# NILOIDE/A.I.gar

Measured on NVIDIA B200. Metric: env_steps_per_sec, higher is better.
Workload: dtype f64

## Files before the change

a.i.gar_b200/csrc/agar_b200.cu:

```cuda
#include <cuda_runtime.h>
#include <math.h>
#include <stdio.h>
#include <stdlib.h>
#include <string.h>

#include "../../include/agar_b200.h"
#include "../../include/agar_layout.h"
#include "agar_bots.cuh"
#include "agar_dev.cuh"
#include "agar_simple.cuh"

extern __shared__ __align__(16) uint8_t g_smem[];

__device__ __forceinline__ void stage_in(const DevParams& P, const uint8_t* state, int env0, int n_here, bool zero) {
    const int chunks = (int)(P.L.record_bytes / 8);
    const int total = n_here * chunks;
    const uint2* src = (const uint2*)(state + (size_t)env0 * P.L.record_bytes);
    for (int i = threadIdx.x; i < total; i += blockDim.x) {
        int e = i / chunks, w = i - e * chunks;
        uint2 v = zero ? make_uint2(0u, 0u) : src[i];
        ((uint2*)(g_smem + (size_t)e * P.rec_stride))[w] = v;
    }
    __syncthreads();
}
// ... 139 lines not shown
            CLK_MARK(1);
            c.fov_done = false, c.n_live = -1;
            for (int ph = 0; ph < AGAR_FIELD_PHASES; ++ph) {
                if (ph == 0 ? psync : psync_field) __syncthreads();
                if (ph == 0) CLK_MARK(2);
                if (active) field_update_phase<W, FULL>(c, P, ph);
                CLK_MARK(3 + ph);
            }
            if (active) {
                if (c.lane == 0) c.h->frame += 1;
                c.t.sync();
            }
            CLK_MARK(12);
        }
        if (active && c.lane == 0 && (P.turn_reward || P.turn_done))
            for (int a = 0; a < A; ++a) {
                if (P.turn_reward) P.turn_reward[(size_t)env * A + a] = (float)c.pl[a].bot.last_reward;
                if (P.turn_done) P.turn_done[(size_t)env * A + a] = (uint8_t)c.pl[a].bot.exp_done;
            }
    }
    if (P.stage == 1) stage_out(P, state, env0, n_here);
    if (P.stage >= 2) {
        __syncthreads();
        pel_cache_copy(P, state, env0, n_here, tiles, false);
    }
    export_tail(P, obs, env0, n_here);
}


struct SimplePlan {
    int frame_sync;
    int strideB;
    int grid_off;
};
template <int W>
__global__ void __launch_bounds__(256, W == 1 ? 2 : 1)
k_simple(const __grid_constant__ DevParams P, const SimplePlan SP, uint8_t* __restrict__ state, const float* __restrict__ actions,
         float* __restrict__ obs, int n_frames, int n_dec, int flags, uint32_t dec_base) {
    const int per = blockDim.x / W;
    const int env0 = blockIdx.x * per;
    const int n_here = min(per, P.n_envs - env0);
    const int rec_words = (int)(P.L.record_bytes / 4), pel_word = (int)(P.L.off_pellets / 4);
    const int tail_words = rec_words - pel_word;
    {
        for (int i = threadIdx.x; i < per * tail_words; i += blockDim.x) {
            int e = i / tail_words, w = i - e * tail_words;
            int es = e < n_here ? e : n_here - 1;
            const uint32_t* src = (const uint32_t*)(state + (size_t)(env0 + es) * P.L.record_bytes) + pel_word;
            *(uint32_t*)(g_smem + (size_t)e * SP.strideB + w * 4) = src[w];
        }
    }
    __syncthreads();
    const int slot = threadIdx.x / W, sub = threadIdx.x % W;
    const bool valid = slot < n_here;
    const int env = env0 + (valid ? slot : n_here - 1);
    const uint32_t env_id = (uint32_t)(P.first_env + (uint64_t)env);
    uint8_t* rec = state + (size_t)env * P.L.record_bytes;
    uint8_t* b = g_smem + (size_t)slot * SP.strideB;
    SPtr q;
    q.h = (AgarEnvHeader*)(rec + P.L.off_header);
    q.p = (AgarPlayer*)(rec + P.L.off_players);
    q.c = (AgarCell*)(rec + P.L.off_cells);
    q.pel = (uint32_t*)b;
    q.ev = (AgarEvent*)(b + (P.L.off_events - P.L.off_pellets));
    q.grid = SP.grid_off ? (uint32_t*)(b + SP.grid_off) : nullptr;
    SReg r;
    s_load(r, q);
    float* row = (obs != nullptr && valid) ? obs + (size_t)env * P.L.state_len : nullptr;
    for (int d = 0; d < n_dec; ++d) {
        if (flags & KF_OBS_BEFORE) {
            int d_o = s_turn_begin(r, P);
            s_observe<W>(r, q, P, d_o != 0, row, sub);
        }
        for (int f = 0; f < n_frames; ++f) {
            if (SP.frame_sync == 1 || SP.frame_sync == 4) __syncthreads();
            if (SP.frame_sync == 2) __syncwarp();
            r.n_events = 0;
            int d_o = s_turn_begin(r, P);
            s_observe<W>(r, q, P, d_o != 0, nullptr, sub);
            float act[4] = {0.f, 0.f, 0.f, 0.f};
            if (r.need_action) {
                if (flags & KF_RANDOM_ACTIONS) {
                    uint32_t w[4];
                    philox(dec_base + (uint32_t)d, 7u, env_id, 0u, (uint32_t)P.seed, (uint32_t)(P.seed >> 32), w);
                    for (int i = 0; i < 4; ++i) act[i] = (float)(w[i] >> 8) * (1.0f / 16777216.0f);
                } else {
                    const float* ap = actions + (size_t)env * 4;
                    for (int i = 0; i < 4; ++i) act[i] = ap[i];
                }
            }
            double speed_pow;
            s_turn_end<W>(r, P, act, sub, speed_pow);
            if (SP.frame_sync == 4) __syncthreads();
            s_field_update<W>(r, q, P, env_id, sub, speed_pow);
        }
    }
    if (flags & KF_OBS_AFTER) {
        int d_o = s_turn_begin(r, P);
        s_observe<W>(r, q, P, d_o != 0, row, sub);
    }
    if (valid && sub == 0) {
        s_store(r, q);
        if (P.turn_reward) P.turn_reward[env] = (float)r.last_reward;
        if (P.turn_done) P.turn_done[env] = (uint8_t)r.exp_done;
    }
    __syncthreads();
    for (int i = threadIdx.x; i < n_here * tail_words; i += blockDim.x) {
        int e = i / tail_words, w = i - e * tail_words;
        uint32_t* dst = (uint32_t*)(state + (size_t)(env0 + e) * P.L.record_bytes) + pel_word;
        dst[w] = *(const uint32_t*)(g_smem + (size_t)e * SP.strideB + w * 4);
    }
    export_tail(P, obs, env0, n_here);
}

template <int W, bool FULL>
__global__ void __launch_bounds__(1024)
k_init(const __grid_constant__ DevParams P, uint8_t* __restrict__ state, const uint8_t* __restrict__ mask, int mode) {
    const int tiles = blockDim.x / W;
    const int env0 = blockIdx.x * tiles;
    const int n_here = min(tiles, P.n_envs - env0);
    if (P.stage == 1)
        stage_in(P, state, env0, n_here, mode == 0);
    else if (mode == 0) {
        const int chunks = (int)(P.L.record_bytes / 8);
        uint2* dst = (uint2*)(state + (size_t)env0 * P.L.record_bytes);
        for (int i = threadIdx.x; i < n_here * chunks; i += blockDim.x) dst[i] = make_uint2(0u, 0u);
        __syncthreads();
    }
    if (P.stage >= 2) pel_cache_copy(P, state, env0, n_here, tiles, true);
    const int tile_id = threadIdx.x / W;
    if (tile_id < n_here && (mask == nullptr || mode == 0 || mask[env0 + tile_id])) {
        Ctx<W> c(cg::tiled_partition<W>(cg::this_thread_block()));
        bind_ctx(c, P, tile_id, tiles, env0 + tile_id, state);
        const int K = P.L.n_players;
        if (mode == 0 || mode == 1) {
            if (mode == 1) {
                for (int i = c.lane; i < P.L.pellet_cap; i += W) c.pel[i] = 0;
// ... 64 lines not shown
    case AGAR_GET_VALID: ((uint8_t*)out)[i] = (uint8_t)p->bot.exp_valid; break;
    case AGAR_GET_NEED_ACTION: ((uint8_t*)out)[i] = (uint8_t)p->bot.need_action; break;
    case AGAR_GET_MASS: {
        int nc = p->n_cells;
        ((float*)out)[i] = nc ? (float)np_sum([&](int j) { return cells[j].mass; }, nc) : 0.f;
        break;
    }
    case AGAR_GET_FOV: ((float*)out)[i] = (float)p->fov_size; break;
    case AGAR_GET_NCELLS: ((int32_t*)out)[i] = p->n_cells; break;
    case AGAR_GET_ALIVE: ((uint8_t*)out)[i] = (uint8_t)p->alive; break;
    case AGAR_GET_STATS: {
        double* o = (double*)out + (size_t)i * 4;
        o[0] = p->bot.stat_mass_sum, o[1] = p->bot.stat_mass_max, o[2] = p->bot.stat_frames, o[3] = p->bot.stat_deaths;
        break;
    }
    case AGAR_GET_OVERFLOW: ((uint32_t*)out)[i] = h->overflow; break;
    case AGAR_GET_EVENT_HASH: ((uint64_t*)out)[i] = h->event_hash; break;
    }
}

struct AgarEnv {
    AgarConfig cfg;
    AgarLayout L;
    DevParams P;
    uint8_t* state;
    double* deg_tab;
    int n_envs, device, W, full, threads, tiles;
    size_t smem_bytes;
    int init_W, init_threads, init_tiles;
    size_t init_smem;
    SimplePlan sp;
    int simple_W, simple_threads;
    size_t simple_smem;
    int64_t launches;
    char err[256];
    float *d_actions, *d_obs, *d_reward;
    uint8_t* d_done;
    void* h_turn;
    volatile uint32_t* h_flag;
    unsigned int* d_export_count;
    uint32_t flag_seq;
    int host_polling;
    int host_pending;
    int host_zerocopy;
};
static char g_create_err[256] = "";

static int fail(AgarEnv* e, int code, const char* fmt, const char* detail) {
    char* dst = e ? e->err : g_create_err;
    snprintf(dst, 256, fmt, detail);
    return code;
}
#define CU(call)                                                                 \
    do {                                                                         \
        cudaError_t _e = (call);                                                 \
        if (_e != cudaSuccess) return fail(env, AGAR_E_CUDA, "CUDA error: %s", cudaGetErrorString(_e)); \
    } while (0)

extern "C" int agar_layout_for_config(const AgarConfig* cfg, AgarLayout* out) {
    if (!cfg || !out) return AGAR_E_INVALID;
    return agar_layout_compute(cfg, out);
}

static bool config_is_simple(const AgarConfig& c, const AgarLayout& L) {
    return c.n_players == 1 && c.bot_type[0] == AGAR_BOT_NN && !c.virus_enabled && !c.enable_split && !c.enable_eject &&
           L.cell_cap == 1 && !c.self_grid && !c.wall_grid && !c.enemy_grid && !c.virus_grid && !c.self_grid_lf &&
           !c.self_grid_slf && !c.enemy_grid_lf && !c.enemy_grid_slf && !c.use_last_action && !c.use_second_last_action &&
// ... 52 lines not shown
    k_main<W, FULL, MAXT><<<blocks, e->threads, e->smem_bytes, s>>>(e->P, e->state, actions, obs, n_frames, n_dec, flags, dec_base);
    return cudaGetLastError();
}
template <int W, bool FULL>
static cudaError_t launch_main_t(AgarEnv* e, const float* actions, float* obs, int n_frames, int n_dec, int flags,
                                 uint32_t dec_base, cudaStream_t s) {
    if (W == 32 && FULL && e->threads > 768) return launch_main_k<32, true, 1024>(e, actions, obs, n_frames, n_dec, flags, dec_base, s);
    if (W == 32 && FULL && e->threads > 512) return launch_main_k<32, true, 768>(e, actions, obs, n_frames, n_dec, flags, dec_base, s);
    return launch_main_k<W, FULL, 512>(e, actions, obs, n_frames, n_dec, flags, dec_base, s);
}
template <int W, bool FULL>
static cudaError_t launch_init_t(AgarEnv* e, const uint8_t* mask, int mode, cudaStream_t s) {
    static unsigned char done[64];
    cudaError_t err = ensure_max_smem(k_init<W, FULL>, e->device, done);
    if (err != cudaSuccess) return err;
    int blocks = (e->n_envs + e->init_tiles - 1) / e->init_tiles;
    k_init<W, FULL><<<blocks, e->init_threads, e->init_smem, s>>>(e->P, e->state, mask, mode);
    return cudaGetLastError();
}
#define DISPATCH(fn, ...)                                                 \
    (e->full ? (e->W == 32  ? fn<32, true>(__VA_ARGS__)                   \
                : e->W == 16 ? fn<16, true>(__VA_ARGS__)                  \
                : e->W == 8  ? fn<8, true>(__VA_ARGS__)                   \
                             : fn<4, true>(__VA_ARGS__))                  \
             : (e->W == 32  ? fn<32, false>(__VA_ARGS__)                  \
                             : fn<32, false>(__VA_ARGS__)))

static int launch_main(AgarEnv* e, const float* actions, float* obs, int n_frames, int n_dec, int flags, uint32_t dec_base,
                       void* stream) {
    AgarEnv* env = e;
    CU(cudaSetDevice(e->device));
    cudaError_t err;
    if (e->simple_W) {
        int blocks = (e->n_envs * e->simple_W + e->simple_threads - 1) / e->simple_threads;
#define LAUNCH_SIMPLE(WW)                                                                                                     \
    do {                                                                                                                      \
        static unsigned char done_##WW[64];                                                                                   \
        err = ensure_max_smem(k_simple<WW>, e->device, done_##WW);                                                            \
        if (err == cudaSuccess) {                                                                                             \
            k_simple<WW><<<blocks, e->simple_threads, e->simple_smem, (cudaStream_t)stream>>>(e->P, e->sp, e->state, actions, obs, \
                                                                                              n_frames, n_dec, flags, dec_base);  \
            err = cudaGetLastError();                                                                                         \
        }                                                                                                                     \
    } while (0)
        if (e->simple_W == 1) LAUNCH_SIMPLE(1);
        else if (e->simple_W == 2) LAUNCH_SIMPLE(2);
        else if (e->simple_W == 4) LAUNCH_SIMPLE(4);
        else if (e->simple_W == 8) LAUNCH_SIMPLE(8);
        else if (e->simple_W == 16) LAUNCH_SIMPLE(16);
        else LAUNCH_SIMPLE(32);
#undef LAUNCH_SIMPLE
    } else
        err = DISPATCH(launch_main_t, e, actions, obs, n_frames, n_dec, flags, dec_base, (cudaStream_t)stream);
    if (err != cudaSuccess) return fail(e, AGAR_E_CUDA, "kernel launch failed: %s", cudaGetErrorString(err));
    e->launches += 1;
    return AGAR_OK;
}
static int launch_init(AgarEnv* e, const uint8_t* mask, int mode, void* stream) {
    AgarEnv* env = e;
    CU(cudaSetDevice(e->device));
    cudaError_t err = e->full ? (e->init_W == 32 ? launch_init_t<32, true>(e, mask, mode, (cudaStream_t)stream)
                                                  : launch_init_t<8, true>(e, mask, mode, (cudaStream_t)stream))
                              : launch_init_t<32, false>(e, mask, mode, (cudaStream_t)stream);
    if (err != cudaSuccess) return fail(e, AGAR_E_CUDA, "kernel launch failed: %s", cudaGetErrorString(err));
    e->launches += 1;
    return AGAR_OK;
}

extern "C" int agar_set_tile_width(AgarEnv* e, int W) {
    if (!e) return AGAR_E_INVALID;
    if (!e->full && e->L.grid_squares <= 16 && (W == 1 || W == 2 || W == 4 || W == 8 || W == 16 || W == 32) &&
        !getenv("AGAR_GENERAL_KERNEL")) {
        int tail_words = (int)((e->L.record_bytes - e->L.off_pellets) / 4);
        e->sp.strideB = (tail_words | 1) * 4;
        e->sp.grid_off = 0;
        const char* genv = getenv("AGAR_SIMPLE_OBS_SMEM");
        if (genv ? atoi(genv) != 0 : W >= 2) {
            const int gg = e->L.grid_squares * e->L.grid_squares;
            e->sp.grid_off = tail_words * 4;
            e->sp.strideB = ((tail_words + gg) | 1) * 4;
        }
        if (e->L.pellet_cap > (W >= 4 ? 64 : 128) * W)
            return fail(e, AGAR_E_UNSUPPORTED, "pellet pool too large for this tile width%s", "");
        int threads = 128;
        const char* tenv = getenv("AGAR_SIMPLE_THREADS");
        if (tenv && atoi(tenv) >= 32) threads = atoi(tenv) / 32 * 32;
        if (threads > 256) threads = 256;
        e->sp.frame_sync = getenv("AGAR_SIMPLE_SYNC") ? atoi(getenv("AGAR_SIMPLE_SYNC")) : 1;
        size_t per_env = (size_t)e->sp.strideB;
        while (threads > 32 && per_env * (threads / W) > 200 * 1024) threads -= 32;
        if (per_env * (threads / W) > 200 * 1024)
            return fail(e, AGAR_E_NOMEM, "pellet pool + event ring of %s do not fit in shared memory at this tile width", "the envs of one CTA");
        e->simple_W = W;
        e->simple_threads = threads;
        e->simple_smem = per_env * (threads / W);
        e->W = W;
        return AGAR_OK;
    }
    bool ok = W == 32 || (e->full && (W == 4 || W == 8 || W == 16));
    if (!ok) return fail(e, AGAR_E_INVALID, "unsupported tile width%s", "");
    if (!plan_launch(e, W)) return fail(e, AGAR_E_NOMEM, "env record does not fit in shared memory%s", "");
    e->simple_W = 0;
    return AGAR_OK;
}
extern "C" int agar_get_tile_width(const AgarEnv* e) { return e ? e->W : 0; }

extern "C" int agar_create(const AgarConfig* cfg, int n_envs, int device, uint64_t seed, uint64_t first_env_id, void* stream,
                           AgarEnv** out) {
    AgarEnv* env = nullptr;
    if (!cfg || !out || n_envs < 1) return fail(nullptr, AGAR_E_INVALID, "bad arguments to agar_create%s", "");
    AgarLayout L;
    int rc = agar_layout_compute(cfg, &L);
    if (rc != AGAR_OK) return fail(nullptr, rc, "config rejected by agar_layout_compute%s", "");
    int ndev = 0;
    if (cudaGetDeviceCount(&ndev) != cudaSuccess || device < 0 || device >= ndev)
        return fail(nullptr, AGAR_E_CUDA, "no such CUDA device%s", "");
    CU(cudaSetDevice(device));
    AgarEnv* e = (AgarEnv*)calloc(1, sizeof(AgarEnv));
    env = e;
    e->cfg = *cfg;
    e->L = L;
    e->n_envs = n_envs;
    e->device = device;
    e->full = config_is_simple(*cfg, L) ? 0 : 1;
    DevParams& P = e->P;
    memset(&P, 0, sizeof P);
    P.cfg = *cfg;
    P.L = L;
    P.S = L.field_size;
// ... 62 lines not shown
        cudaFree(e->state), cudaFree(e->deg_tab), free(e);
        return AGAR_E_NOMEM;
    }
    rc = launch_init(e, nullptr, 0, stream);
    if (rc != AGAR_OK) {
        snprintf(g_create_err, sizeof g_create_err, "%s", e->err);
        cudaFree(e->state), cudaFree(e->deg_tab), free(e);
        return rc;
    }
    *out = e;
    return AGAR_OK;
}
extern "C" int agar_destroy(AgarEnv* e) {
    if (!e) return AGAR_E_INVALID;
    cudaSetDevice(e->device);
    cudaFree(e->state);
    cudaFree(e->deg_tab);
    if (e->d_actions) cudaFree(e->d_actions);
    if (e->d_obs) cudaFree(e->d_obs);
    if (e->d_reward) cudaFree(e->d_reward);
    if (e->h_turn) cudaFreeHost(e->h_turn);
    if (e->d_export_count) cudaFree(e->d_export_count);
    free(e);
    return AGAR_OK;
}
extern "C" const char* agar_last_error(const AgarEnv* e) { return e ? e->err : g_create_err; }
extern "C" int agar_get_layout(const AgarEnv* e, AgarLayout* out) {
    if (!e || !out) return AGAR_E_INVALID;
    *out = e->L;
    return AGAR_OK;
}
extern "C" int agar_num_envs(const AgarEnv* e) { return e ? e->n_envs : AGAR_E_INVALID; }
extern "C" int64_t agar_launch_count(const AgarEnv* e) { return e ? e->launches : 0; }
extern "C" void* agar_state_ptr(const AgarEnv* e) { return e ? e->state : nullptr; }

extern "C" int agar_reset(AgarEnv* e, const uint8_t* env_mask_dev, void* stream) {
    if (!e) return AGAR_E_INVALID;
    return launch_init(e, env_mask_dev, 1, stream);
}
extern "C" int agar_reset_bots(AgarEnv* e, const uint8_t* env_mask_dev, void* stream) {
    if (!e) return AGAR_E_INVALID;
    return launch_init(e, env_mask_dev, 2, stream);
}
extern "C" int agar_observe(AgarEnv* e, float* obs_dev, void* stream) {
    if (!e) return AGAR_E_INVALID;
    return launch_main(e, nullptr, obs_dev, 0, 0, KF_OBS_AFTER, 0, stream);
}
extern "C" int agar_step(AgarEnv* e, const float* actions_dev, int n_frames, void* stream) {
    if (!e || n_frames < 0) return AGAR_E_INVALID;
    if (!actions_dev && e->L.n_agents > 0) return fail(e, AGAR_E_INVALID, "actions_dev is NULL%s", "");
    return launch_main(e, actions_dev, nullptr, n_frames, 1, 0, 0, stream);
}
extern "C" int agar_step_observe(AgarEnv* e, const float* actions_dev, int n_frames, float* obs_dev, void* stream) {
    if (!e || n_frames < 0) return AGAR_E_INVALID;
    if (!actions_dev && e->L.n_agents > 0) return fail(e, AGAR_E_INVALID, "actions_dev is NULL%s", "");
    return launch_main(e, actions_dev, obs_dev, n_frames, 1, KF_OBS_AFTER, 0, stream);
}
extern "C" int agar_rollout_random(AgarEnv* e, int n_decisions, int n_frames, uint32_t decision_base, float* obs_dev,
                                   void* stream) {
    if (!e || n_decisions < 0 || n_frames < 0) return AGAR_E_INVALID;
    return launch_main(e, nullptr, obs_dev, n_frames, n_decisions, KF_OBS_BEFORE | KF_RANDOM_ACTIONS, decision_base, stream);
}
extern "C" int agar_get(AgarEnv* e, AgarField which, void* out_dev, void* stream) {
    AgarEnv* env = e;
    if (!e || !out_dev || (int)which < 0 || (int)which > AGAR_GET_EVENT_HASH) return AGAR_E_INVALID;
    CU(cudaSetDevice(e->device));
// ... 129 lines not shown
```

a.i.gar_b200/csrc/agar_simple.cuh:

```cuda
#pragma once
#include "agar_bots.cuh"
#include "agar_dev.cuh"

#define S_FULL 0xffffffffu
#define S_NONE 0x7fffffff

struct SReg {
    uint32_t rng_field, frame;
    int32_t n_pellets, n_events;
    uint64_t event_hash;
    double cmd_x, cmd_y, fov_x, fov_y, fov_size;
    int32_t fov_valid;
    double x, y, mass, radius, svx, svy, merge_time;
    int32_t counter;
    uint32_t uid, flags;
    int32_t has_action, has_last_action, skip_frames, has_last_mass, has_old_state, time, skipping, turn_begun, need_action,
        exp_valid, exp_done;
    double a0, a1, a2, a3, l0, l1, l2, l3;
    double cum_reward, last_reward, last_mass, fov_size_feat, stat_mass_sum, stat_mass_max, stat_frames;
};

struct SPtr {
    AgarEnvHeader* h;
    AgarPlayer* p;
// ... 120 lines not shown
            r.fov_y = fy;
            r.fov_valid = 1;
        }
    }
    const double mass_next = r.mass >= 4 ? r.mass * P.decay_rate : r.mass;
    double fov_pow;
    s_dual_pow<W>(r.radius, 0.475, mass_next, -0.35, sub, fov_pow, speed_pow);
    r.fov_size = fov_pow * P.pow_n[1] * 35;
    int x = (int)r.fov_x, y = (int)r.fov_y;
    int left = x - (int)(r.fov_size / 2), top = y - (int)(r.fov_size / 2);
    int size = (int)r.fov_size;
    r.cmd_x = left + a0 * size;
    r.cmd_y = top + a1 * size;
}

template <int W>
struct SMask {
    typedef uint32_t T;
    static constexpr int MB = 32;
};
template <>
struct SMask<1> {
    typedef unsigned long long T;
    static constexpr int MB = 64;
};
template <>
struct SMask<2> {
    typedef unsigned long long T;
    static constexpr int MB = 64;
};
DEV int s_ffs(uint32_t m) { return __ffs((int)m); }
DEV int s_ffs(unsigned long long m) { return __ffsll((long long)m); }

template <int W>
DEV void s_observe(SReg& r, const SPtr& q, const DevParams& P, bool mine, float* row, int sub) {
    const int G = P.L.grid_squares, GG = G * G, SL = P.L.state_len;
    const double S = (double)P.S;
    if (mine) {
        s_update_fov(r, P);
        r.fov_size_feat = P.cfg.use_fovsize ? r.fov_size : r.fov_size_feat;
    }
    const bool out = mine && row != nullptr;
    if (!s_any<W>(out)) return;
    const bool staged = q.grid != nullptr;
    if (out) {
        if (staged)
            for (int i = sub; i < GG; i += W) q.grid[i] = 0u;
        else
            for (int i = sub; i < GG; i += W) row[i] = 0.f;
        if (sub == 0) {
            int n = GG;
            if (P.cfg.use_fovsize) row[n++] = (float)r.fov_size;
            if (P.cfg.use_totalmass) row[n++] = (float)(0.0 + r.mass);
            (void)SL;
        }
    }
    s_sync<W>();
    if (out) {
        const double fov = r.fov_size, fx = r.fov_x, fy = r.fov_y;
        const double left = fx - fov / 2, top = fy - fov / 2;
        const double gs = fov / G, inv = 1.0 / gs;
        const bool canon = P.cfg.obs_mode == AGAR_OBS_CANONICAL;
        const int cols = canon ? G : (int)ceil(fov / gs);
        double mx = left + gs / 2, my = top + gs / 2;
        unsigned col_bad = 0, row_bad = 0;
        for (int i = 0; i < G; ++i) {
            if (mx + gs / 2 < 0 || mx - gs / 2 > S) col_bad |= 1u << i;
            if (my + gs / 2 < 0 || my - gs / 2 > S) row_bad |= 1u << i;
            mx += gs;
            my += gs;
        }
        const Rect ra = rect_of(P.S, fx, fy, fov / 2);
        const double h = fov / 2;
        const double xmin = fx - h, xmax = fx + h, ymin = fy - h, ymax = fy + h;
        const int wx0 = (int)floor(xmin) - 1, wx1 = (int)ceil(xmax) + 1, wy0 = (int)floor(ymin) - 1, wy1 = (int)ceil(ymax) + 1;
// ... 35 lines not shown
            double dx = (double)px, dy = (double)py;
            bool ok = rect_hit(ra, pellet_rect(px, py)) && !(dx + pr < xmin || dx - pr > xmax || dy + pr < ymin || dy - pr > ymax);
            int c0, c1, r0, r1;
            if (use_bits) {
                axis_buckets2_bits(dx - left, pr, fov, gs, inv, edges, c0, c1);
                axis_buckets2_bits(dy - top, pr, fov, gs, inv, edges, r0, r1);
            } else {
                axis_buckets2(dx - left, pr, fov, gs, inv, canon, c0, c1);
                axis_buckets2(dy - top, pr, fov, gs, inv, canon, r0, r1);
            }
            float fm = (float)pm;
            auto put = [&](int cc, int rr) {
                int sr = sheared ? cc + rr : cc, sc = rr;
                if (sr >= G) sr -= G, sc += 1;
                int id = sr + sc * G;
                if (ok && cc >= 0 && rr >= 0 && sc < G && !((row_bad >> sc & 1) || (col_bad >> sr & 1))) {
                    if (staged)
                        atomicAdd(&q.grid[id], (unsigned)pm);
                    else
                        atomicAdd(&row[id], fm);
                }
            };
            put(c0, r0);
            put(c1, r0);
            put(c0, r1);
            put(c1, r1);
        }
    }
    if (staged) {
        s_sync<W>();
        if (out)
            for (int i = sub; i < GG; i += W) row[i] = (float)q.grid[i];
    }
}

template <int W>
DEV void s_field_update(SReg& r, const SPtr& q, const DevParams& P, uint32_t env_id, int sub, double speed_pow) {
    const double S = (double)P.S;
    double mass = r.mass, radius = r.radius;
    if (mass >= 4) {
        mass = mass * P.decay_rate;
        radius = radius_of(mass);
    }
    update_momentum(r.svx, r.svy, r.counter);
    if (r.merge_time > 0) r.merge_time = r.merge_time - 1;
    double xd = r.cmd_x - r.x, yd = r.cmd_y - r.y;
    double h2 = xd * xd + yd * yd, r2 = radius * radius;
    double sm = (h2 < r2 ? h2 : r2) / r2;
    double cs, sn;
    agar_dir(yd, xd, &cs, &sn);
    double rs = P.move_speed * speed_pow;
    double vx = rs * sm * cs, vy = rs * sm * sn;
    update_pos(r.x, r.y, vx, vy, r.svx, r.svy, r.counter, S);
    r.flags |= AGAR_CF_INHASH;
    const double radius0 = radius;
    const double cx = r.x, cy = r.y;
    const int cap = P.L.pellet_cap;
    constexpr bool DISC = W >= 4;
    const int icx = (int)cx, icy = (int)cy;
    int reach = (int)radius + 1;
    const float cxf = (float)cx, cyf = (float)cy;
    float thr = 0.9101f * (float)(radius * radius) + 0.1f;
    const bool pool_full = r.n_pellets == cap;
    int eaten0 = S_NONE, eaten1 = S_NONE, eaten2 = S_NONE, eaten3 = S_NONE, n_eaten = 0;
    typedef typename SMask<W>::T MT;
    constexpr int MB = SMask<W>::MB;
// ... 145 lines not shown
```

a.i.gar_b200/env.py:

```python
import ctypes
import os

import numpy as np

from . import layout as lay

_HERE = os.path.dirname(os.path.abspath(__file__))
_LIB_PATH = os.environ.get("AGAR_B200_LIB", os.path.join(_HERE, "libagar_b200.so"))
_lib = None

EXPORTS = ["agar_layout_for_config", "agar_create", "agar_destroy", "agar_last_error", "agar_get_layout", "agar_num_envs",
           "agar_reset", "agar_reset_bots", "agar_observe", "agar_step", "agar_step_observe", "agar_get",
           "agar_debug_dump", "agar_debug_load", "agar_launch_count", "agar_step_host", "agar_rollout_random",
           "agar_set_tile_width", "agar_get_tile_width", "agar_state_ptr",
           "agar_step_host_begin", "agar_step_host_end"]


def load_library():
    global _lib
    if _lib is not None:
        return _lib
    if not os.path.exists(_LIB_PATH):
        raise ImportError("%s not found: build it with `python -m aigar_b200.build` (needs nvcc); "
                          "there is no CPU fallback" % _LIB_PATH)
# ... 66 lines not shown
        self.actions = torch.zeros((self.n_envs, max(a, 1), 4), dtype=torch.float32, device=self.device)

    def _stream(self):
        if self.stream is not None:
            return ctypes.c_void_p(self.stream.cuda_stream)
        return ctypes.c_void_p(self.torch.cuda.current_stream(self.device).cuda_stream)

    def _check(self, rc):
        if rc != 0:
            raise AgarError("agar call failed (%d): %s" % (rc, self.lib.agar_last_error(self.h).decode()))

    def close(self):
        if getattr(self, "h", None) and self.h.value:
            self.lib.agar_destroy(self.h)
            self.h = ctypes.c_void_p()

    def __del__(self):
        try:
            self.close()
        except Exception:
            pass

    @property
    def tile_width(self):
        return self.lib.agar_get_tile_width(self.h)

    def set_tile_width(self, w):
        self._check(self.lib.agar_set_tile_width(self.h, int(w)))

    @property
    def launch_count(self):
        return int(self.lib.agar_launch_count(self.h))

    def _ptr(self, t):
        return ctypes.c_void_p(t.data_ptr()) if t is not None else ctypes.c_void_p()

    def _actions(self, actions):
        if actions is None:
            return self.actions
        t = self.torch.as_tensor(actions, dtype=self.torch.float32, device=self.device)
        t = t.reshape(self.n_envs, max(self.layout.n_agents, 1), 4).contiguous()
        return t

    def reset(self, mask=None):
        m = None if mask is None else self.torch.as_tensor(mask, dtype=self.torch.uint8, device=self.device).contiguous()
        self._check(self.lib.agar_reset(self.h, self._ptr(m), self._stream()))

    def reset_bots(self, mask=None):
        m = None if mask is None else self.torch.as_tensor(mask, dtype=self.torch.uint8, device=self.device).contiguous()
        self._check(self.lib.agar_reset_bots(self.h, self._ptr(m), self._stream()))

    def observe(self, out=None):
        out = self.obs if out is None else out
        self._check(self.lib.agar_observe(self.h, self._ptr(out), self._stream()))
        return out

    def step(self, actions=None, n_frames=1):
        a = self._actions(actions)
        self._check(self.lib.agar_step(self.h, self._ptr(a), int(n_frames), self._stream()))

    def step_observe(self, actions=None, n_frames=1, out=None):
        a = self._actions(actions)
        out = self.obs if out is None else out
        self._check(self.lib.agar_step_observe(self.h, self._ptr(a), int(n_frames), self._ptr(out), self._stream()))
        return out

# ... 100 lines not shown
```

include/agar_b200.h:

```cpp
#ifndef AGAR_B200_H
#define AGAR_B200_H

#include <stdint.h>
#include <stddef.h>

#ifdef __cplusplus
extern "C" {
#endif

#define AGAR_ABI_VERSION 1

#define AGAR_MAX_PLAYERS 16
#define AGAR_MAX_CELLS   16
#define AGAR_ACTION_DIM  4

enum { AGAR_OK = 0, AGAR_E_INVALID = -1, AGAR_E_CUDA = -2, AGAR_E_NOMEM = -3, AGAR_E_UNSUPPORTED = -4,
       AGAR_E_RANGE = -5 };

enum { AGAR_BOT_NN = 0, AGAR_BOT_GREEDY = 1, AGAR_BOT_RANDOM = 2 };

enum { AGAR_OBS_REFERENCE = 0, AGAR_OBS_CANONICAL = 1 };
#define AGAR_SIMPLE_STATE_LEN 12

typedef struct AgarConfig {
// ... 169 lines not shown
typedef struct AgarEnv AgarEnv;

int agar_layout_for_config(const AgarConfig* cfg, AgarLayout* out);

int agar_create(const AgarConfig* cfg, int n_envs, int device, uint64_t seed, uint64_t first_env_id, void* stream,
                AgarEnv** out);
int agar_destroy(AgarEnv* env);
const char* agar_last_error(const AgarEnv* env);
int agar_get_layout(const AgarEnv* env, AgarLayout* out);
int agar_num_envs(const AgarEnv* env);

int agar_reset(AgarEnv* env, const uint8_t* env_mask_dev, void* stream);
int agar_reset_bots(AgarEnv* env, const uint8_t* env_mask_dev, void* stream);

int agar_observe(AgarEnv* env, float* obs_dev, void* stream);

int agar_step(AgarEnv* env, const float* actions_dev, int n_frames, void* stream);

int agar_step_observe(AgarEnv* env, const float* actions_dev, int n_frames, float* obs_dev, void* stream);

int agar_rollout_random(AgarEnv* env, int n_decisions, int n_frames, uint32_t decision_base, float* obs_dev,
                        void* stream);

int agar_get(AgarEnv* env, AgarField which, void* out_dev, void* stream);

int agar_set_tile_width(AgarEnv* env, int lanes);
int agar_get_tile_width(const AgarEnv* env);
void* agar_state_ptr(const AgarEnv* env);

int agar_debug_dump(AgarEnv* env, int env_index, void* record_host, size_t bytes, void* stream);
int agar_debug_load(AgarEnv* env, int env_index, const void* record_host, size_t bytes, void* stream);

int64_t agar_launch_count(const AgarEnv* env);

int agar_step_host(AgarEnv* env, const float* actions_host, int n_frames, float* obs_host, float* reward_host,
                   uint8_t* done_host, void* stream);
int agar_step_host_begin(AgarEnv* env, const float* actions_host, int n_frames, float* obs_host, void* stream);
int agar_step_host_end(AgarEnv* env, float* reward_host, uint8_t* done_host, void* stream);

#ifdef __cplusplus
}
#endif
#endif
```

Baseline: 955.1 million.

## Add producer-consumer observer warps to overlap observation encoding with physics

Adds dedicated observer warps to the simple kernel. Physics threads snapshot per-env FOV and pellet state into double-buffered shared memory each decision, and the observer warps encode observations from those snapshots, synchronised with named barriers. The goal is to take observation encoding off the physics critical path when observing before actions with enough frames per decision. It costs extra shared memory and threads per block, and a host-side occupancy check falls back to the old path when the new shape would need more waves.

```diff
diff --git a/a.i.gar_b200/csrc/agar_b200.cu b/a.i.gar_b200/csrc/agar_b200.cu
--- a/a.i.gar_b200/csrc/agar_b200.cu
+++ b/a.i.gar_b200/csrc/agar_b200.cu
@@ -195,12 +195,33 @@
     int frame_sync;
     int strideB;
     int grid_off;
+    int obs_warps;
+    int snap_off;
+    int snap_stride;
 };
-template <int W>
-__global__ void __launch_bounds__(256, W == 1 ? 2 : 1)
+
+enum { SB_PHYS = 1, SB_FULL = 2, SB_EMPTY = 4 };
+struct SimpleSnap {
+    double fov_x, fov_y, fov_size, mass;
+    int32_t out;
+    int32_t pad;
+};
+__host__ __device__ constexpr int simple_max_threads(int W) { return W == 8 ? 352 : 256; }
+constexpr int SIMPLE_OBS_MIN_FRAMES = 4;
+constexpr int SIMPLE_OBS_LANES = 4;
+constexpr int SIMPLE_OBS_WARPS = 4;
+
+template <int ID>
+DEV void named_bar_sync(int n) { asm volatile("bar.sync %0, %1;" ::"n"(ID), "r"(n) : "memory"); }
+template <int ID>
+DEV void named_bar_arrive(int n) { asm volatile("bar.arrive %0, %1;" ::"n"(ID), "r"(n) : "memory"); }
+
+template <int W, bool OBSW>
+__global__ void __launch_bounds__(OBSW ? simple_max_threads(W) : 256, W == 1 ? 2 : 1)
 k_simple(const __grid_constant__ DevParams P, const SimplePlan SP, uint8_t* __restrict__ state, const float* __restrict__ actions,
          float* __restrict__ obs, int n_frames, int n_dec, int flags, uint32_t dec_base) {
-    const int per = blockDim.x / W;
+    const int phys_threads = blockDim.x - 32 * SP.obs_warps;
+    const int per = phys_threads / W;
     const int env0 = blockIdx.x * per;
     const int n_here = min(per, P.n_envs - env0);
     const int rec_words = (int)(P.L.record_bytes / 4), pel_word = (int)(P.L.off_pellets / 4);
@@ -214,58 +235,108 @@
         }
     }
     __syncthreads();
-    const int slot = threadIdx.x / W, sub = threadIdx.x % W;
-    const bool valid = slot < n_here;
-    const int env = env0 + (valid ? slot : n_here - 1);
-    const uint32_t env_id = (uint32_t)(P.first_env + (uint64_t)env);
-    uint8_t* rec = state + (size_t)env * P.L.record_bytes;
-    uint8_t* b = g_smem + (size_t)slot * SP.strideB;
-    SPtr q;
-    q.h = (AgarEnvHeader*)(rec + P.L.off_header);
-    q.p = (AgarPlayer*)(rec + P.L.off_players);
-    q.c = (AgarCell*)(rec + P.L.off_cells);
-    q.pel = (uint32_t*)b;
-    q.ev = (AgarEvent*)(b + (P.L.off_events - P.L.off_pellets));
-    q.grid = SP.grid_off ? (uint32_t*)(b + SP.grid_off) : nullptr;
-    SReg r;
-    s_load(r, q);
-    float* row = (obs != nullptr && valid) ? obs + (size_t)env * P.L.state_len : nullptr;
-    for (int d = 0; d < n_dec; ++d) {
-        if (flags & KF_OBS_BEFORE) {
+    auto snap = [&](int buf, int e) { return g_smem + SP.snap_off + (size_t)(buf * per + e) * SP.snap_stride; };
+    if (OBSW && (int)threadIdx.x >= phys_threads) {
+        constexpr int WO = SIMPLE_OBS_LANES;
+        const int ot = ((int)threadIdx.x - phys_threads) / WO, osub = threadIdx.x % WO, n_ot = 32 * SP.obs_warps / WO;
+        for (int d = 0; d < n_dec; ++d) {
+            const int buf = d & 1;
+            if (buf) named_bar_sync<SB_FULL + 1>(blockDim.x);
+            else named_bar_sync<SB_FULL>(blockDim.x);
+            for (int base = 0; base < per; base += n_ot) {
+                const int e = min(base + ot, per - 1);
+                const SimpleSnap* sn = (const SimpleSnap*)snap(buf, e);
+                SReg r;
+                r.fov_x = sn->fov_x, r.fov_y = sn->fov_y, r.fov_size = sn->fov_size, r.mass = sn->mass;
+                SPtr q;
+                q.pel = (uint32_t*)(sn + 1);
+                q.grid = (uint32_t*)(g_smem + (size_t)e * SP.strideB + SP.grid_off);
+                const bool out = base + ot < per && sn->out != 0;
+                s_encode<WO>(r, q, P, out, out ? obs + (size_t)(env0 + e) * P.L.state_len : nullptr, osub);
+            }
+            if (d + 2 < n_dec) {
+                if (buf) named_bar_arrive<SB_EMPTY + 1>(blockDim.x);
+                else named_bar_arrive<SB_EMPTY>(blockDim.x);
+            }
+        }
+        if (flags & KF_OBS_AFTER) __syncthreads();
+    } else {
+        const int slot = threadIdx.x / W, sub = threadIdx.x % W;
+        const bool valid = slot < n_here;
+        const int env = env0 + (valid ? slot : n_here - 1);
+        const uint32_t env_id = (uint32_t)(P.first_env + (uint64_t)env);
+        uint8_t* rec = state + (size_t)env * P.L.record_bytes;
+        uint8_t* b = g_smem + (size_t)slot * SP.strideB;
+        SPtr q;
+        q.h = (AgarEnvHeader*)(rec + P.L.off_header);
+        q.p = (AgarPlayer*)(rec + P.L.off_players);
+        q.c = (AgarCell*)(rec + P.L.off_cells);
+        q.pel = (uint32_t*)b;
+        q.ev = (AgarEvent*)(b + (P.L.off_events - P.L.off_pellets));
+        q.grid = SP.grid_off ? (uint32_t*)(b + SP.grid_off) : nullptr;
+        SReg r;
+        s_load(r, q);
+        float* row = (obs != nullptr && valid) ? obs + (size_t)env * P.L.state_len : nullptr;
+        auto frame_bar = [&]() {
+            if (OBSW) named_bar_sync<SB_PHYS>(phys_threads);
+            else __syncthreads();
+        };
+        for (int d = 0; d < n_dec; ++d) {
+            if (OBSW && SP.obs_warps) {
+                const int d_o = s_turn_begin(r, P);
+                if (d_o) s_observe_state(r, P);
+                const int buf = d & 1;
+                if (d >= 2) {
+                    if (buf) named_bar_sync<SB_EMPTY + 1>(blockDim.x);
+                    else named_bar_sync<SB_EMPTY>(blockDim.x);
+                }
+                uint8_t* sn = snap(buf, slot);
+                uint32_t* pool = (uint32_t*)(sn + sizeof(SimpleSnap));
+                for (int i = sub; i < P.L.pellet_cap; i += W) pool[i] = q.pel[i];
+                if (sub == 0) {
+                    SimpleSnap* h = (SimpleSnap*)sn;
+                    h->fov_x = r.fov_x, h->fov_y = r.fov_y, h->fov_size = r.fov_size, h->mass = r.mass;
+                    h->out = d_o != 0 && row != nullptr;
+                }
+                if (buf) named_bar_arrive<SB_FULL + 1>(blockDim.x);
+                else named_bar_arrive<SB_FULL>(blockDim.x);
+            } else if (flags & KF_OBS_BEFORE) {
+                int d_o = s_turn_begin(r, P);
+                s_observe<W>(r, q, P, d_o != 0, row, sub);
+            }
+            for (int f = 0; f < n_frames; ++f) {
+                if (SP.frame_sync == 1 || SP.frame_sync == 4) frame_bar();
+                if (SP.frame_sync == 2) __syncwarp();
+                r.n_events = 0;
+                int d_o = s_turn_begin(r, P);
+                s_observe<W>(r, q, P, d_o != 0, nullptr, sub);
+                float act[4] = {0.f, 0.f, 0.f, 0.f};
+                if (r.need_action) {
+                    if (flags & KF_RANDOM_ACTIONS) {
+                        uint32_t w[4];
+                        philox(dec_base + (uint32_t)d, 7u, env_id, 0u, (uint32_t)P.seed, (uint32_t)(P.seed >> 32), w);
+                        for (int i = 0; i < 4; ++i) act[i] = (float)(w[i] >> 8) * (1.0f / 16777216.0f);
+                    } else {
+                        const float* ap = actions + (size_t)env * 4;
+                        for (int i = 0; i < 4; ++i) act[i] = ap[i];
+                    }
+                }
+                double speed_pow;
+                s_turn_end<W>(r, P, act, sub, speed_pow);
+                if (SP.frame_sync == 4) frame_bar();
+                s_field_update<W>(r, q, P, env_id, sub, speed_pow);
+            }
+        }
+        if (flags & KF_OBS_AFTER) {
+            if (OBSW) __syncthreads();
             int d_o = s_turn_begin(r, P);
             s_observe<W>(r, q, P, d_o != 0, row, sub);
         }
-        for (int f = 0; f < n_frames; ++f) {
-            if (SP.frame_sync == 1 || SP.frame_sync == 4) __syncthreads();
-            if (SP.frame_sync == 2) __syncwarp();
-            r.n_events = 0;
-            int d_o = s_turn_begin(r, P);
-            s_observe<W>(r, q, P, d_o != 0, nullptr, sub);
-            float act[4] = {0.f, 0.f, 0.f, 0.f};
-            if (r.need_action) {
-                if (flags & KF_RANDOM_ACTIONS) {
-                    uint32_t w[4];
-                    philox(dec_base + (uint32_t)d, 7u, env_id, 0u, (uint32_t)P.seed, (uint32_t)(P.seed >> 32), w);
-                    for (int i = 0; i < 4; ++i) act[i] = (float)(w[i] >> 8) * (1.0f / 16777216.0f);
-                } else {
-                    const float* ap = actions + (size_t)env * 4;
-                    for (int i = 0; i < 4; ++i) act[i] = ap[i];
-                }
-            }
-            double speed_pow;
-            s_turn_end<W>(r, P, act, sub, speed_pow);
-            if (SP.frame_sync == 4) __syncthreads();
-            s_field_update<W>(r, q, P, env_id, sub, speed_pow);
-        }
-    }
-    if (flags & KF_OBS_AFTER) {
-        int d_o = s_turn_begin(r, P);
-        s_observe<W>(r, q, P, d_o != 0, row, sub);
-    }
-    if (valid && sub == 0) {
-        s_store(r, q);
-        if (P.turn_reward) P.turn_reward[env] = (float)r.last_reward;
-        if (P.turn_done) P.turn_done[env] = (uint8_t)r.exp_done;
+        if (valid && sub == 0) {
+            s_store(r, q);
+            if (P.turn_reward) P.turn_reward[env] = (float)r.last_reward;
+            if (P.turn_done) P.turn_done[env] = (uint8_t)r.exp_done;
+        }
     }
     __syncthreads();
     for (int i = threadIdx.x; i < n_here * tail_words; i += blockDim.x) {
@@ -396,7 +467,11 @@
     SimplePlan sp;
     int simple_W, simple_threads;
     size_t simple_smem;
+    SimplePlan sp_obs;
+    int obs_threads;
+    size_t obs_smem;
     int64_t launches;
+    int64_t observer_launches;
     char err[256];
     float *d_actions, *d_obs, *d_reward;
     uint8_t* d_done;
@@ -515,24 +590,35 @@
     CU(cudaSetDevice(e->device));
     cudaError_t err;
     if (e->simple_W) {
-        int blocks = (e->n_envs * e->simple_W + e->simple_threads - 1) / e->simple_threads;
-#define LAUNCH_SIMPLE(WW)                                                                                                     \
+        const bool handoff = e->obs_threads && (flags & KF_OBS_BEFORE) && obs != nullptr && n_frames >= SIMPLE_OBS_MIN_FRAMES;
+        const SimplePlan& sp = handoff ? e->sp_obs : e->sp;
+        const int threads = handoff ? e->obs_threads : e->simple_threads;
+        const size_t smem = handoff ? e->obs_smem : e->simple_smem;
+        const int per = (threads - 32 * sp.obs_warps) / e->simple_W;
+        if (threads % 32 || threads > (handoff ? simple_max_threads(e->simple_W) : 256) || per < 1 || per * e->simple_W % 32 ||
+            (sp.obs_warps && (!sp.grid_off || 32 * sp.obs_warps % SIMPLE_OBS_LANES)))
+            return fail(e, AGAR_E_INVALID, "inconsistent k_simple launch shape%s", "");
+        int blocks = (e->n_envs + per - 1) / per;
+#define LAUNCH_SIMPLE(WW, OB)                                                                                                 \
     do {                                                                                                                      \
-        static unsigned char done_##WW[64];                                                                                   \
-        err = ensure_max_smem(k_simple<WW>, e->device, done_##WW);                                                            \
+        static unsigned char done_##WW##OB[64];                                                                               \
+        err = ensure_max_smem(k_simple<WW, OB>, e->device, done_##WW##OB);                                                    \
         if (err == cudaSuccess) {                                                                                             \
-            k_simple<WW><<<blocks, e->simple_threads, e->simple_smem, (cudaStream_t)stream>>>(e->P, e->sp, e->state, actions, obs, \
-                                                                                              n_frames, n_dec, flags, dec_base);  \
+            k_simple<WW, OB><<<blocks, threads, smem, (cudaStream_t)stream>>>(e->P, sp, e->state, actions, obs, n_frames,     \
+                                                                              n_dec, flags, dec_base);                        \
             err = cudaGetLastError();                                                                                         \
         }                                                                                                                     \
     } while (0)
-        if (e->simple_W == 1) LAUNCH_SIMPLE(1);
-        else if (e->simple_W == 2) LAUNCH_SIMPLE(2);
-        else if (e->simple_W == 4) LAUNCH_SIMPLE(4);
-        else if (e->simple_W == 8) LAUNCH_SIMPLE(8);
-        else if (e->simple_W == 16) LAUNCH_SIMPLE(16);
-        else LAUNCH_SIMPLE(32);
+        if (handoff && e->simple_W == 4) LAUNCH_SIMPLE(4, true);
+        else if (handoff) LAUNCH_SIMPLE(8, true);
+        else if (e->simple_W == 1) LAUNCH_SIMPLE(1, false);
+        else if (e->simple_W == 2) LAUNCH_SIMPLE(2, false);
+        else if (e->simple_W == 4) LAUNCH_SIMPLE(4, false);
+        else if (e->simple_W == 8) LAUNCH_SIMPLE(8, false);
+        else if (e->simple_W == 16) LAUNCH_SIMPLE(16, false);
+        else LAUNCH_SIMPLE(32, false);
 #undef LAUNCH_SIMPLE
+        if (handoff && err == cudaSuccess) e->observer_launches += 1;
     } else
         err = DISPATCH(launch_main_t, e, actions, obs, n_frames, n_dec, flags, dec_base, (cudaStream_t)stream);
     if (err != cudaSuccess) return fail(e, AGAR_E_CUDA, "kernel launch failed: %s", cudaGetErrorString(err));
@@ -550,6 +636,54 @@
     return AGAR_OK;
 }
 
+template <int W, bool OBSW>
+static int simple_ctas_per_sm(int device, int threads, size_t smem) {
+    static unsigned char done[64];
+    int n = 0;
+    if (ensure_max_smem(k_simple<W, OBSW>, device, done) != cudaSuccess ||
+        cudaOccupancyMaxActiveBlocksPerMultiprocessor(&n, k_simple<W, OBSW>, threads, smem) != cudaSuccess) {
+        cudaGetLastError();
+        return 0;
+    }
+    return n;
+}
+
+static void plan_observers(AgarEnv* e) {
+    e->obs_threads = 0;
+    e->sp_obs = e->sp;
+    const int W = e->simple_W;
+    if ((W != 4 && W != 8) || !e->sp.grid_off || e->L.pellet_cap > 64 * SIMPLE_OBS_LANES) return;
+    if (cudaSetDevice(e->device) != cudaSuccess) {
+        cudaGetLastError();
+        return;
+    }
+    int sms = 148;
+    cudaDeviceGetAttribute(&sms, cudaDevAttrMultiProcessorCount, e->device);
+    const int per_warp = 32 / W;
+    const int K = SIMPLE_OBS_WARPS;
+    int warps = ((e->n_envs + sms - 1) / sms + per_warp - 1) / per_warp;
+    if (warps > simple_max_threads(W) / 32 - K) warps = simple_max_threads(W) / 32 - K;
+    const int per = warps * per_warp;
+    const size_t env_bytes = ((size_t)per * e->sp.strideB + 15) / 16 * 16;
+    const int snap_stride = (int)((sizeof(SimpleSnap) + (size_t)e->L.pellet_cap * 4 + 15) / 16 * 16);
+    const size_t smem = env_bytes + 2 * (size_t)per * snap_stride;
+    if (smem > 200 * 1024) return;
+    const int threads = (warps + K) * 32;
+    const int occ = W == 8 ? simple_ctas_per_sm<8, true>(e->device, threads, smem) : simple_ctas_per_sm<4, true>(e->device, threads, smem);
+    const int occ_in = W == 8 ? simple_ctas_per_sm<8, false>(e->device, e->simple_threads, e->simple_smem)
+                              : simple_ctas_per_sm<4, false>(e->device, e->simple_threads, e->simple_smem);
+    if (occ < 1 || occ_in < 1) return;
+    const long long per_in = e->simple_threads / W;
+    const long long waves = ((e->n_envs + per - 1) / per + (long long)sms * occ - 1) / ((long long)sms * occ);
+    const long long waves_in = ((e->n_envs + per_in - 1) / per_in + (long long)sms * occ_in - 1) / ((long long)sms * occ_in);
+    if (waves > waves_in) return;
+    e->sp_obs.obs_warps = K;
+    e->sp_obs.snap_off = (int)env_bytes;
+    e->sp_obs.snap_stride = snap_stride;
+    e->obs_threads = threads;
+    e->obs_smem = smem;
+}
+
 extern "C" int agar_set_tile_width(AgarEnv* e, int W) {
     if (!e) return AGAR_E_INVALID;
     if (!e->full && e->L.grid_squares <= 16 && (W == 1 || W == 2 || W == 4 || W == 8 || W == 16 || W == 32) &&
@@ -557,6 +691,7 @@
         int tail_words = (int)((e->L.record_bytes - e->L.off_pellets) / 4);
         e->sp.strideB = (tail_words | 1) * 4;
         e->sp.grid_off = 0;
+        e->sp.obs_warps = e->sp.snap_off = e->sp.snap_stride = 0;
         const char* genv = getenv("AGAR_SIMPLE_OBS_SMEM");
         if (genv ? atoi(genv) != 0 : W >= 2) {
             const int gg = e->L.grid_squares * e->L.grid_squares;
@@ -578,6 +713,7 @@
         e->simple_threads = threads;
         e->simple_smem = per_env * (threads / W);
         e->W = W;
+        plan_observers(e);
         return AGAR_OK;
     }
     bool ok = W == 32 || (e->full && (W == 4 || W == 8 || W == 16));
@@ -706,6 +842,7 @@
 }
 extern "C" int agar_num_envs(const AgarEnv* e) { return e ? e->n_envs : AGAR_E_INVALID; }
 extern "C" int64_t agar_launch_count(const AgarEnv* e) { return e ? e->launches : 0; }
+extern "C" int64_t agar_observer_launch_count(const AgarEnv* e) { return e ? e->observer_launches : 0; }
 extern "C" void* agar_state_ptr(const AgarEnv* e) { return e ? e->state : nullptr; }
 
 extern "C" int agar_reset(AgarEnv* e, const uint8_t* env_mask_dev, void* stream) {
diff --git a/a.i.gar_b200/csrc/agar_simple.cuh b/a.i.gar_b200/csrc/agar_simple.cuh
--- a/a.i.gar_b200/csrc/agar_simple.cuh
+++ b/a.i.gar_b200/csrc/agar_simple.cuh
@@ -176,15 +176,15 @@
 DEV int s_ffs(uint32_t m) { return __ffs((int)m); }
 DEV int s_ffs(unsigned long long m) { return __ffsll((long long)m); }
 
-template <int W>
-DEV void s_observe(SReg& r, const SPtr& q, const DevParams& P, bool mine, float* row, int sub) {
+DEV void s_observe_state(SReg& r, const DevParams& P) {
+    s_update_fov(r, P);
+    r.fov_size_feat = P.cfg.use_fovsize ? r.fov_size : r.fov_size_feat;
+}
+
+template <int W>
+DEV void s_encode(const SReg& r, const SPtr& q, const DevParams& P, bool out, float* row, int sub) {
     const int G = P.L.grid_squares, GG = G * G, SL = P.L.state_len;
     const double S = (double)P.S;
-    if (mine) {
-        s_update_fov(r, P);
-        r.fov_size_feat = P.cfg.use_fovsize ? r.fov_size : r.fov_size_feat;
-    }
-    const bool out = mine && row != nullptr;
     if (!s_any<W>(out)) return;
     const bool staged = q.grid != nullptr;
     if (out) {
@@ -286,6 +286,12 @@
         if (out)
             for (int i = sub; i < GG; i += W) row[i] = (float)q.grid[i];
     }
+}
+
+template <int W>
+DEV void s_observe(SReg& r, const SPtr& q, const DevParams& P, bool mine, float* row, int sub) {
+    if (mine) s_observe_state(r, P);
+    s_encode<W>(r, q, P, mine && row != nullptr, row, sub);
 }
 
 template <int W>
diff --git a/a.i.gar_b200/env.py b/a.i.gar_b200/env.py
--- a/a.i.gar_b200/env.py
+++ b/a.i.gar_b200/env.py
@@ -122,6 +122,12 @@
     def launch_count(self):
         return int(self.lib.agar_launch_count(self.h))
 
+    @property
+    def observer_launch_count(self):
+        fn = self.lib.agar_observer_launch_count
+        fn.argtypes, fn.restype = [ctypes.c_void_p], ctypes.c_int64
+        return int(fn(self.h))
+
     def _ptr(self, t):
         return ctypes.c_void_p(t.data_ptr()) if t is not None else ctypes.c_void_p()
 
diff --git a/include/agar_b200.h b/include/agar_b200.h
--- a/include/agar_b200.h
+++ b/include/agar_b200.h
@@ -225,6 +225,7 @@
 int agar_debug_load(AgarEnv* env, int env_index, const void* record_host, size_t bytes, void* stream);
 
 int64_t agar_launch_count(const AgarEnv* env);
+int64_t agar_observer_launch_count(const AgarEnv* env);
 
 int agar_step_host(AgarEnv* env, const float* actions_host, int n_frames, float* obs_host, float* reward_host,
                    uint8_t* done_host, void* stream);
```

Measured after the change: 1.124 billion (median of 6 runs). +17.7%, better.
